# SarahAlkhateeb/Image-Captioning-with-Different-Decoders

Hardware: AMD Instinct MI355X
Metric: training images/sec (whole node), 'attention' decoder, at 1/2/4/8 MI355X (higher is better)
Workload: dtype fp32; 1 GPU; 'attention' decoder + frozen ResNet-101 encoder (BN train mode), one training step per batch; per_gpu_batch=64, global_batch=64, image_size=224, caption_len=25, decode_steps=24, vocab=8100, attention_dim=512, decoder_dim=512, embed_size=512, decoder_rows=49 distinct (AdaptiveAvgPool 7->14 replicate; exact, DESIGN.md 4.4), parallelism=dp1

## Files before the change

### image-captioning-with-different-decoders_amd/capmi/_lib.py

```python
import ctypes
import os

import torch

_HERE = os.path.dirname(os.path.abspath(__file__))
LIB_PATH = os.environ.get("CAPMI_LIB") or os.path.join(_HERE, "libcapmi.so")

c_int, c_ll, c_float, c_double, c_vp = ctypes.c_int, ctypes.c_longlong, ctypes.c_float, ctypes.c_double, ctypes.c_void_p
c_ull = ctypes.c_ulonglong

CAPMI_A_KMAJOR, CAPMI_A_MMAJOR, CAPMI_A_CONV_NHWC, CAPMI_A_CONV_NCHW, CAPMI_A_CONV_NHWC4 = 0, 1, 2, 3, 4
CAPMI_B_NMAJOR_W, CAPMI_B_KROWS, CAPMI_B_CONV_NHWC = 0, 1, 2
CAPMI_TILE_128, CAPMI_TILE_64, CAPMI_TILE_128x64, CAPMI_TILE_AUTO, CAPMI_TILE_128_W8 = 0, 1, 2, 3, 4
CAPMI_MAX_GROUP = 4
CAPMI_COLSUM_GROUPS = 64
ABI_VERSION = 27
CAPMI_BNB_RELU_Y, CAPMI_BNB_RELU_OUT = 0, 1
CAPMI_BNB_MAX_SLABS = 256
CAPMI_GEMM_BF16 = 1
CAPMI_GEMM_BF16_IO = 2
CAPMI_GEMM_X3 = 4
CAPMI_GEMM_X3P = 8
CAPMI_GEMM_SPLIT3 = 16
CAPMI_GEMM_X3D = 32
# ... 28 lines not shown

class DstepEpi(ctypes.Structure):
    _fields_ = [
        ("mode", c_int), ("out0", c_vp), ("ld0", c_ll), ("bias0", c_vp), ("nsplit", c_int),
        ("out1", c_vp), ("ld1", c_ll), ("bias1", c_vp), ("act1", c_int), ("D", c_int),
        ("xemb", c_vp), ("c_prev", c_vp), ("h_out", c_vp), ("c_out", c_vp), ("act_out", c_vp),
        ("dhd", c_vp), ("dc_in", c_vp), ("act", c_vp), ("c_cur", c_vp), ("dgates", c_vp), ("dc_out", c_vp),
        ("bt", c_int), ("gate", c_vp), ("awe", c_vp), ("dawe_out", c_vp), ("dgp", c_vp),
    ]


CAPMI_DSTEP_STORE2, CAPMI_DSTEP_LSTM_FWD, CAPMI_DSTEP_LSTM_BWD, CAPMI_DSTEP_GATE_BWD = 0, 1, 2, 3

_SIGS = {
    "capmi_gemm": [ctypes.POINTER(GemmProblem), c_int, c_int, c_int, c_int, c_vp],
    "capmi_gemm_stat_tiles": [c_int, c_int],
    "capmi_gemm_workspace_bytes": [],
    "capmi_gemm_workspace_flag_bytes": [],
    "capmi_gemm_sk": [ctypes.POINTER(GemmProblem), c_int, c_int, c_int, c_vp, c_ll, c_vp],
    "capmi_gemm_ex": [ctypes.POINTER(GemmProblem), c_int, c_int, c_int, c_int, c_int, c_vp],
    "capmi_gemm_sk_ex": [ctypes.POINTER(GemmProblem), c_int, c_int, c_int, c_int, c_vp, c_ll, c_vp],
    "capmi_gemm_sk_plan": [ctypes.POINTER(GemmProblem), c_int, c_int, c_int, c_int, c_vp, c_vp, c_vp, c_vp, c_vp],
    "capmi_last_launch_name": [ctypes.c_char_p, c_int],
    "capmi_splitk_reduce": [c_vp, c_int, c_ll, c_int, c_int, c_ll, c_vp, c_vp, c_ll, c_vp],
    "capmi_colsum": [c_vp, c_int, c_int, c_ll, c_float, c_vp, c_vp, c_int, c_vp],
    "capmi_conv_weight_pack": [c_vp, c_int, c_int, c_int, c_int, c_vp, c_vp],
    "capmi_conv_weight_pack_pad": [c_vp, c_int, c_int, c_int, c_int, c_int, c_vp, c_vp],
    "capmi_image_nhwc4": [c_vp, c_int, c_int, c_int, c_int, c_vp, c_vp],
    "capmi_bn_finalize": [c_vp, c_int, c_int, c_ll, c_vp, c_vp, c_vp, c_vp, c_float, c_float,
                          c_vp, c_vp, c_vp, c_vp, c_vp, c_vp],
    "capmi_bn_eval_params": [c_vp, c_vp, c_vp, c_vp, c_int, c_float, c_vp, c_vp, c_vp],
    "capmi_bn_add_relu": [c_vp, c_vp, c_vp, c_vp, c_vp, c_vp, c_vp, c_ll, c_int, c_vp],
    "capmi_bn_relu_maxpool": [c_vp, c_vp, c_vp, c_vp, c_int, c_int, c_int, c_int, c_int, c_int, c_vp],
    "capmi_adaptive_avgpool_nhwc": [c_vp, c_int, c_int, c_int, c_int, c_int, c_int, c_vp, c_vp],
    "capmi_conv_weight_pack_dgrad": [c_vp, c_int, c_int, c_int, c_int, c_vp, c_vp],
    "capmi_conv_weight_pack_dgrad_s2": [c_vp, c_int, c_int, c_int, c_int, c_vp, c_vp],
    "capmi_conv_weight_pack_dgrad_x3": [c_vp, c_int, c_int, c_int, c_int, c_int, c_int, c_vp, c_vp],
    "capmi_weight_x3_batch": [c_vp, c_int, c_ll, c_vp],
    "capmi_conv_weight_unpack": [c_vp, c_int, c_int, c_int, c_int, c_vp, c_vp],
    "capmi_zero_upsample2_nhwc": [c_vp, c_int, c_int, c_int, c_int, c_int, c_int, c_vp, c_vp],
    "capmi_bn_bwd_reduce": [c_int, c_vp, c_vp, c_vp, c_vp, c_vp, c_vp, c_vp, c_vp, c_float, c_ll, c_int,
                            c_vp, c_vp, c_int, c_vp, c_vp, c_vp],
    "capmi_bn_bwd_apply": [c_int, c_vp, c_vp, c_vp, c_vp, c_vp, c_vp, c_ll, c_int, c_vp, c_vp, c_vp],
    "capmi_adaptive_avgpool_bwd_nhwc": [c_vp, c_int, c_int, c_int, c_int, c_int, c_int, c_vp, c_vp],
    "capmi_embed_gather": [c_vp, c_int, c_int, c_vp, c_int, c_int, c_int, c_vp, c_ll, c_vp],
    "capmi_embed_dense": [c_vp, c_int, c_int, c_int, c_int, c_vp, c_ll, c_vp],
# ... 111 lines not shown
```

### image-captioning-with-different-decoders_amd/capmi/kernels.py

```python
import ctypes
import weakref

import torch

from ._lib import DstepEpi, DstepSeg
from ._lib import (CAPMI_A_CONV_NHWC, CAPMI_A_KMAJOR, CAPMI_A_MMAJOR, CAPMI_B_NMAJOR_W, CAPMI_BNB_MAX_SLABS, CAPMI_GEMM_BF16,
                   CAPMI_GEMM_BF16_IO, CAPMI_GEMM_X3, CAPMI_GEMM_X3P,
                   CAPMI_GEMM_SPLIT3, CAPMI_GEMM_X3C, CAPMI_GEMM_X3D, CAPMI_GEMM_X3S, CAPMI_GEMM_X3W,
                   CAPMI_COLSUM_GROUPS, CAPMI_TILE_128, CAPMI_TILE_64,
                   CAPMI_TILE_128x64, CAPMI_TILE_AUTO, GemmProblem, call, lib)

F32 = torch.float32


def ptr(t):
    return None if t is None else t.data_ptr()


def stream():
    return torch.cuda.current_stream().cuda_stream


def _cuda(*ts, dtype=F32):
    for t in ts:
# ... 169 lines not shown
    v = [ctypes.c_int(0) for _ in range(5)]
    call("capmi_gemm_sk_plan", ctypes.byref(prob), CAPMI_A_MMAJOR, bmode, CAPMI_TILE_AUTO, _x3w_flags(bf16),
         *[ctypes.byref(x) for x in v])
    return f"{'gemm_w16_kernel' if bf16 else 'gemm_x3w_kernel'}<{bmode}, {'true' if v[2].value else 'false'}>"


def gemm_x3w_ok(prob, bmode, bf16=False):
    v = [ctypes.c_int(0) for _ in range(5)]
    return lib.capmi_gemm_sk_plan(ctypes.byref(prob), CAPMI_A_MMAJOR, bmode, CAPMI_TILE_AUTO, _x3w_flags(bf16),
                                  *[ctypes.byref(x) for x in v]) == 0


def gemm_x3s_ok(prob, amode):
    v = [ctypes.c_int(0) for _ in range(5)]
    return lib.capmi_gemm_sk_plan(ctypes.byref(prob), amode, CAPMI_B_NMAJOR_W, CAPMI_TILE_AUTO, CAPMI_GEMM_X3S,
                                  *[ctypes.byref(x) for x in v]) == 0


def gemm_x3s_kernel_name(prob, amode):
    ncb = {64: 1, 128: 2, 256: 4}[prob.N]
    return f"gemm_x3s_kernel<{ncb}, {'true' if prob.in_scale else 'false'}>"


def gemm_x3d_kernel_name(prob, amode):
    v = [ctypes.c_int(0) for _ in range(5)]
    call("capmi_gemm_sk_plan", ctypes.byref(prob), amode, CAPMI_B_NMAJOR_W, CAPMI_TILE_AUTO, CAPMI_GEMM_X3D,
         *[ctypes.byref(x) for x in v])
    b = lambda x: "true" if x else "false"
    return f"gemm_x3p_kernel<{amode}, {b(v[2].value)}, 32, true, {b(bool(prob.in_scale))}>"


def gemm_x3p_kernel_name(prob, amode):
    v = [ctypes.c_int(0) for _ in range(5)]
    call("capmi_gemm_sk_plan", ctypes.byref(prob), amode, CAPMI_B_NMAJOR_W, CAPMI_TILE_AUTO, CAPMI_GEMM_X3P,
         *[ctypes.byref(x) for x in v])
    return f"gemm_x3p_kernel<{amode}, {'true' if v[2].value else 'false'}, {v[3].value}, false, false>"


def gemm_x3_kernel_name(prob, amode, tile=CAPMI_TILE_AUTO):
    v = [ctypes.c_int(0) for _ in range(5)]
    call("capmi_gemm_sk_plan", ctypes.byref(prob), amode, CAPMI_B_NMAJOR_W, tile, CAPMI_GEMM_X3,
         *[ctypes.byref(x) for x in v])
    b = lambda x: "true" if x else "false"
    return f"gemm_x3_kernel<{v[1].value}, {amode}, {b(bool(prob.in_scale))}, {b(v[2].value)}>"


# ... 621 lines not shown
```

### image-captioning-with-different-decoders_amd/capmi/resnet.py

```python
import os

import torch
import torch.nn as nn

from . import kernels as K
from ._lib import CAPMI_A_CONV_NHWC, CAPMI_A_CONV_NHWC4, CAPMI_A_KMAJOR, CAPMI_A_MMAJOR, CAPMI_B_CONV_NHWC
from ._lib import CAPMI_B_KROWS, CAPMI_B_NMAJOR_W, CAPMI_GEMM_BF16, CAPMI_GEMM_SPLIT3

AK, AMM, AC = CAPMI_A_KMAJOR, CAPMI_A_MMAJOR, CAPMI_A_CONV_NHWC
BW, BKR, BCONV = CAPMI_B_NMAJOR_W, CAPMI_B_KROWS, CAPMI_B_CONV_NHWC


class Bottleneck(nn.Module):
    expansion = 4

    def __init__(self, cin, width, stride=1, downsample=False):
        super().__init__()
        self.conv1 = nn.Conv2d(cin, width, 1, bias=False)
        self.bn1 = nn.BatchNorm2d(width)
        self.conv2 = nn.Conv2d(width, width, 3, stride=stride, padding=1, bias=False)
        self.bn2 = nn.BatchNorm2d(width)
        self.conv3 = nn.Conv2d(width, width * 4, 1, bias=False)
        self.bn3 = nn.BatchNorm2d(width * 4)
        self.relu = nn.ReLU(inplace=True)
# ... 70 lines not shown
        return ent[2]


def feature_hw(H, W):
    def down(x, k, st, pad):
        return (x + 2 * pad - k) // st + 1
    h, w = down(down(H, 7, 2, 3), 3, 2, 1), down(down(W, 7, 2, 3), 3, 2, 1)
    for _ in range(3):
        h, w = down(h, 3, 2, 1), down(w, 3, 2, 1)
    return h, w


def pool_dup(H, W, out_hw):
    fh, fw = feature_hw(H, W)
    oh, ow = out_hw
    if fh <= 0 or fw <= 0 or oh % fh or ow % fw or oh // fh != ow // fw:
        return 1
    return oh // fh


_X3_SMALLK = int(os.environ.get("CAPMI_X3_SMALLK", "0"))
_X3D = os.environ.get("CAPMI_X3D", "1") != "0"
_X3S = os.environ.get("CAPMI_X3S", "1") != "0"
_X3C = os.environ.get("CAPMI_X3C", "1") != "0"

class EncoderRunner:

    def __init__(self):
        self.packed = _Packed()
        self._ws = None
        self._ws_key = None
        self.conv_hook = None
        self.bf16 = False
        self.x3 = False

    def _workspace(self, N, H, W, device):
        key = (N, H, W, str(device))
        if self._ws_key != key:
            H1, W1 = (H + 6 - 7) // 2 + 1, (W + 6 - 7) // 2 + 1
            big = N * H1 * W1 * 64
            big = max(big, N * ((H1 + 1) // 2) * ((W1 + 1) // 2) * 256)
            f = dict(device=device, dtype=torch.float32)
            ws = {n: torch.empty(big, **f) for n in ("x", "y1", "y2", "y3", "yd", "out")}
            ws["stats"] = torch.empty(2 * ((N * H1 * W1 + 63) // 64) * 256, **f)
            ws["bnwork"] = torch.zeros(K.bn_work_doubles(2048), device=device, dtype=torch.float64)
            ws["ss"] = {}
            ws["sk"] = K.gemm_workspace(device)
            ws["img4"] = torch.empty(N * H * W * 4, **f)
            ws["x3p"] = None
            self._ws, self._ws_key = ws, key
        return self._ws

    def _x3p_buffer(self, ws):
        if ws["x3p"] is None:
            ws["x3p"] = torch.empty(3 * ws["x"].numel(), device=ws["x"].device, dtype=torch.bfloat16)
        return ws["x3p"]

# ... 122 lines not shown
            prob = K.problem(rows, co, Kd, x, ci, w, Kd, out, co, **kw_)
            mode = CAPMI_A_KMAJOR
        else:
            sc, sh = in_ss if in_ss is not None else (None, None)
            w = self._packed_x3(conv) if x3 and Kd % 32 == 0 and ci % 32 == 0 else self.packed.get(conv)
            prob = K.problem(rows, co, Kd, x, 0, w, Kd, out, co, conv=geo, in_scale=sc, in_shift=sh, **kw_)
            mode = CAPMI_A_CONV_NHWC
        if w.dtype == torch.bfloat16:
            launch = lambda: K.gemm_x3(prob, mode, self._ws["sk"])
            if self.conv_hook is not None:
                self.conv_hook(tag, 2.0 * rows * co * Kd, launch, K.gemm_x3_kernel_name(prob, mode))
            else:
                launch()
            return Ho, Wo, rows
        flags = CAPMI_GEMM_BF16 if self.bf16 else (CAPMI_GEMM_SPLIT3 if split3 else 0)
        launch = lambda: K.gemm_sk(prob, mode, self._ws["sk"], K.TILE_AUTO, flags=flags)
        if self.conv_hook is not None:
            key = K.gemm_sk_kernel_name(prob, mode, flags=flags)
            self.conv_hook(tag, 2.0 * rows * co * Kd, launch, key)
        else:
            launch()
        del stats
        return Ho, Wo, rows

    def _packed_x3(self, conv, tap_inner=False):
        w = conv.weight
        key = ("x3p" if tap_inner else "x3", id(conv))
        ent = self.packed.cache.get(key)
        if ent is None or ent[0] != w._version or ent[1] != w.data_ptr():
            src = self.packed.get(conv)
            if tap_inner:
                co, ci, kh, kw = w.shape
                src = K.conv_weight_order_x3p(src, kh, kw, ci)
            src = src.contiguous()
            dst = torch.empty(3 * src.numel(), device=w.device, dtype=torch.bfloat16)
            K.split3_bf16(src, dst)
            ent = (w._version, w.data_ptr(), dst)
            self.packed.cache[key] = ent
        return ent[2]

    def _packed_bf16(self, conv):
        w = conv.weight
        key = ("bf16", id(conv))
        ent = self.packed.cache.get(key)
        if ent is None or ent[0] != w._version or ent[1] != w.data_ptr():
            src = self.packed.get(conv).contiguous()
# ... 83 lines not shown
        N, C0, H, W = imgs.shape
        if self.bf16:
            return self._forward_bf16(net, imgs, out_hw, train, out)
        ws = self._workspace(N, H, W, imgs.device)
        H1, W1, rows = self._conv("conv1", imgs, net.conv1, ws["y1"], N, H, W, train, nchw=True)
        s, b = self._bn(ws, net.bn1, rows, train)
        Hp, Wp = (H1 + 2 - 3) // 2 + 1, (W1 + 2 - 3) // 2 + 1
        K.bn_relu_maxpool(ws["y1"], s, b, ws["x"], N, H1, W1, 64, Hp, Wp)
        x, xo = ws["x"], ws["out"]
        H, W, Cx = Hp, Wp, 64
        bns = []
        direct = out_hw is None and out is not None
        n4 = len(net.layer4)
        for li in range(1, 5):
            layer = getattr(net, f"layer{li}")
            for bi, blk in enumerate(layer):
                if direct and li == 4 and bi == n4 - 1:
                    xo = out
                tag = f"layer{li}.{bi}"
                _, _, r1 = self._conv(tag + ".conv1", x, blk.conv1, ws["y1"], N, H, W, train)
                ss1 = self._bn(ws, blk.bn1, r1, train)
                H2, W2, r2 = self._conv(tag + ".conv2", ws["y1"], blk.conv2, ws["y2"], N, H, W, train, in_ss=ss1)
                ss2 = self._bn(ws, blk.bn2, r2, train)
                _, _, r3 = self._conv(tag + ".conv3", ws["y2"], blk.conv3, ws["y3"], N, H2, W2, train, in_ss=ss2)
                Cout = blk.conv3.out_channels
                if blk.downsample is not None:
                    s3, b3 = self._bn(ws, blk.bn3, r3, train)
                    self._conv(tag + ".downsample", x, blk.downsample[0], ws["yd"], N, H, W, train)
                    sd, bd = self._bn(ws, blk.downsample[1], r3, train)
                    K.bn_add_relu(ws["y3"], s3, b3, ws["yd"], xo, r3, Cout, res_scale=sd, res_shift=bd)
                    bns.append(blk.downsample[1])
                else:
                    s3, b3 = self._bn(ws, blk.bn3, r3, train)
                    K.bn_add_relu(ws["y3"], s3, b3, x, xo, r3, Cout)
                bns += [blk.bn1, blk.bn2, blk.bn3]
                x, xo = xo, x
                H, W, Cx = H2, W2, Cout
        if train:
            bns.append(net.bn1)
            nbt = [m.num_batches_tracked for m in bns if m.num_batches_tracked is not None]
            if nbt:
                torch._foreach_add_(nbt, 1)
        if out_hw is None:
            return x if direct else x[: N * H * W * Cx].view(N, H, W, Cx).clone()
        OH, OW = out_hw
        if out is None:
            out = torch.empty(N, OH, OW, Cx, device=imgs.device, dtype=torch.float32)
        K.adaptive_avgpool_nhwc(x, N, H, W, Cx, OH, OW, out)
        return out


def conv_flops_per_image(net, H=224, W=224):
    tot = 0
    h, w = H, W
    convs = [net.conv1]
# ... 99 lines not shown
        for li in range(1, 5):
            for bi, blk in enumerate(getattr(net, f"layer{li}")):
                tag = f"layer{li}.{bi}"
                wd, Cout = blk.conv1.out_channels, blk.conv3.out_channels
                st = blk.conv2.stride[0]
                H2, W2 = (H + 2 - 3) // st + 1, (W + 2 - 3) // st + 1
                r1, r3 = N * H * W, N * H2 * W2
                if li < self.first:
                    y1, y2, y3, yd, o = ws["y1"], ws["y2"], ws["y3"], ws["yd"], xo
                else:
                    g = self.saved.get
                    y1 = g(tag + ".y1", r1 * wd, dev)
                    y2 = g(tag + ".y2", r3 * wd, dev)
                    y3 = g(tag + ".y3", r3 * Cout, dev)
                    yd = g(tag + ".yd", r3 * Cout, dev) if blk.downsample is not None else None
                    o = g(tag + ".out", r3 * Cout, dev)
                trainable = li >= self.first
                bnf = (lambda bn, rows: self._bn_save(ws, bn, rows)) if trainable else \
                    (lambda bn, rows: r._bn(ws, bn, rows, True) + (None,))
                r._conv(tag + ".conv1", x, blk.conv1, y1, N, H, W, True)
                s1, b1, m1 = bnf(blk.bn1, r1)
                r._conv(tag + ".conv2", y1, blk.conv2, y2, N, H, W, True, in_ss=(s1, b1))
                s2, b2, m2 = bnf(blk.bn2, r3)
                r._conv(tag + ".conv3", y2, blk.conv3, y3, N, H2, W2, True, in_ss=(s2, b2))
                s3, b3, m3 = bnf(blk.bn3, r3)
                md = sd = bd = None
                if blk.downsample is not None:
                    r._conv(tag + ".downsample", x, blk.downsample[0], yd, N, H, W, True)
                    sd, bd, md = bnf(blk.downsample[1], r3)
                    K.bn_add_relu(y3, s3, b3, yd, o, r3, Cout, res_scale=sd, res_shift=bd)
                    bns.append(blk.downsample[1])
                else:
                    K.bn_add_relu(y3, s3, b3, x, o, r3, Cout)
                bns += [blk.bn1, blk.bn2, blk.bn3]
                if trainable:
                    blocks.append(dict(blk=blk, tag=tag, li=li, x=x, Cin=Cx, H=H, W=W, H2=H2, W2=W2, wd=wd, Cout=Cout,
                                       stride=st, y1=y1, y2=y2, y3=y3, yd=yd, out=o,
                                       ss=[(s1, b1, m1), (s2, b2, m2), (s3, b3, m3), (sd, bd, md)]))
                    x = o
                else:
                    x, xo = o, x
                H, W, Cx = H2, W2, Cout
        nbt = [m.num_batches_tracked for m in bns if m.num_batches_tracked is not None]
        if nbt:
            torch._foreach_add_(nbt, 1)
        OH, OW = out_hw if out_hw is not None else (H, W)
        if out is None:
            out = torch.empty(N, OH, OW, Cx, device=dev, dtype=torch.float32)
        K.adaptive_avgpool_nhwc(x, N, H, W, Cx, OH, OW, out)
        self.state = dict(N=N, H=H, W=W, C=Cx, OH=OH, OW=OW, blocks=blocks, device=dev)
        return out

    def _flags(self, prob, amode, bmode):
        if not (self.r.x3 and _FT_DGRAD_X3):
            return 0
# ... 275 lines not shown
```

### image-captioning-with-different-decoders_amd/csrc/gemm.hip

```cpp
#include <cstdlib>

#include "common.h"

#include "gemm_args.h"

constexpr int BK = 16;

template <int AMODE> struct APad { static constexpr int v = 2; };
template <> struct APad<1> { static constexpr int v = 4; };
template <> struct APad<3> { static constexpr int v = 4; };
template <int BMODE> struct BPad { static constexpr int v = 2; };
template <> struct BPad<1> { static constexpr int v = 4; };

template <bool VEC>
__device__ __forceinline__ float4 load4(const float* p, int n) {
  if (VEC) {
    return n > 0 ? *reinterpret_cast<const float4*>(p) : make_float4(0.f, 0.f, 0.f, 0.f);
  } else {
    float4 v = make_float4(0.f, 0.f, 0.f, 0.f);
    if (n > 0) v.x = p[0];
    if (n > 1) v.y = p[1];
    if (n > 2) v.z = p[2];
    if (n > 3) v.w = p[3];
    return v;
// ... 1094 lines not shown
                CAPMI_ERANGE);
  CAPMI_REQUIRE(gemm_x3c_band_fits(p), CAPMI_EINVAL);
  tiles = (int)cdiv(p.M, 256);
  return 0;
}

int gemm_x3c(const capmi_gemm_problem* prob, int amode, int bmode, hipStream_t s) {
  int tiles = 0;
  const int rc = x3c_plan(prob, amode, bmode, tiles);
  if (rc) return rc;
  if (prob->M == 0) return 0;
  return gemm_x3c_launch(*prob, tiles, s);
}

int gemm_x3s(const capmi_gemm_problem* prob, int amode, int bmode, hipStream_t s) {
  long long lda = 0;
  int tiles = 0, grid = 0;
  const int rc = x3s_plan(prob, amode, bmode, lda, tiles, grid);
  if (rc) return rc;
  if (prob->M == 0) return 0;
  return gemm_x3s_launch(*prob, lda, tiles, grid, s);
}

int gemm_x3(const capmi_gemm_problem* prob, int amode, int bmode, int tile, void* workspace, long long ws_bytes,
            hipStream_t s) {
  GemmArgs a;
  int bn = 128;
  bool sk = false;
  long long total = 0;
  const int rc = x3_plan(prob, amode, bmode, tile, a, bn, sk, total);
  if (rc) return rc;
  if (prob->M == 0) return 0;
  if (!sk || workspace == nullptr) return gemm_x3_launch(a, amode, bn, (int)total, s);
  CAPMI_REQUIRE(aligned16(workspace), CAPMI_EINVAL);
  CAPMI_REQUIRE(ws_bytes >= capmi_gemm_workspace_bytes(), CAPMI_ERANGE);
  const int cus = cu_count();
  const long long slots = sk_cus();
  a.sk_nkt = prob->K / 32;
  a.sk_dp_tiles = sk_hybrid() && total >= 2 * slots ? (int)((total / slots - 1) * slots) : 0;
  a.sk_units = (total - a.sk_dp_tiles) * a.sk_nkt;
  a.sk_workers = (int)std::min<long long>(slots, a.sk_units);
  a.sk_groups = sk_xcd_groups() && a.sk_workers % 8 == 0 && total >= 64 ? 8 : 1;
  a.sk_flags = static_cast<int*>(workspace);
  a.sk_part = reinterpret_cast<float*>(static_cast<char*>(workspace) + sk_flag_bytes(cus));
  return gemm_x3_launch(a, amode, bn, a.sk_workers, s);
}
}

extern "C" int capmi_gemm_sk_ex(const capmi_gemm_problem* prob, int amode, int bmode, int tile, int flags,
                                void* workspace, long long ws_bytes, void* stream) {
  GemmPlan g;
  bool sk = false;
  if (flags == CAPMI_GEMM_BF16_IO) return gemm_bf16_io(prob, amode, bmode, tile, workspace, ws_bytes, as_stream(stream));
  if (flags == CAPMI_GEMM_X3) return gemm_x3(prob, amode, bmode, tile, workspace, ws_bytes, as_stream(stream));
  if (flags == CAPMI_GEMM_X3P) return gemm_x3p(prob, amode, bmode, workspace, ws_bytes, as_stream(stream));
  if (flags == CAPMI_GEMM_X3D) return gemm_x3d(prob, amode, bmode, workspace, ws_bytes, as_stream(stream));
  if (flags == CAPMI_GEMM_X3S) return gemm_x3s(prob, amode, bmode, as_stream(stream));
  if (flags == CAPMI_GEMM_X3W) return gemm_x3w(prob, amode, bmode, workspace, ws_bytes, as_stream(stream), 3);
  if (flags == (CAPMI_GEMM_X3W | CAPMI_GEMM_BF16))
    return gemm_x3w(prob, amode, bmode, workspace, ws_bytes, as_stream(stream), 1);
  if (flags == CAPMI_GEMM_X3C) return gemm_x3c(prob, amode, bmode, as_stream(stream));
  int terms = flag_terms(flags);
  CAPMI_REQUIRE(terms >= 0, CAPMI_EINVAL);
  CAPMI_REQUIRE(terms_mode_ok(terms, amode, bmode), CAPMI_EINVAL);
  int rc = sk_decide(prob, amode, bmode, tile, terms, g, sk);
  if (rc) return rc;
  if (terms > 0 && !(g.nt_ok && g.nt == 256 && (prob->in_scale == nullptr || amode == CAPMI_A_CONV_NHWC || bmode == CAPMI_B_CONV_NHWC))) {
    terms = 0;
    rc = sk_decide(prob, amode, bmode, tile, 0, g, sk);
    if (rc) return rc;
  }
// ... 93 lines not shown
```

### image-captioning-with-different-decoders_amd/csrc/gemm_args.h

```cpp
#pragma once
#include "common.h"

typedef float f32x16 __attribute__((ext_vector_type(16)));

struct GemmArgs {
  capmi_gemm_problem p[CAPMI_MAX_GROUP];
  int tiles_begin[CAPMI_MAX_GROUP + 1];
  int tiles_m[CAPMI_MAX_GROUP];
  int tiles_n[CAPMI_MAX_GROUP];
  int kchunk[CAPMI_MAX_GROUP];
  int nprob;
  int sk_workers;
  int sk_nkt;
  long long sk_units;
  int sk_dp_tiles;
  int sk_groups;
  float* sk_part;
  int* sk_flags;
  int tile_cols_first;
  int plain_epi;
  int x3d_pipe;
};

typedef float capmi_f32x2 __attribute__((ext_vector_type(2)));
// ... 43 lines not shown

__device__ __forceinline__ long long remap(long long r, long long r1, long long ld, long long s2) {
  return r1 > 0 ? (r % r1) * ld + (r / r1) * s2 : r * ld;
}

inline int plain_epilogue(const capmi_gemm_problem& p, int bn) {
  static const bool off = [] {
    const char* e = getenv("CAPMI_X3_PLAIN_EPI");
    return e && e[0] == '0';
  }();
  const bool ok = !off && p.alpha == 1.f && p.alpha_ptr == nullptr && p.bias == nullptr && p.bias2 == nullptr &&
                  !p.relu && p.c_r1 <= 0 && p.ksplit == 1 && p.N % bn == 0 && p.ldc >= p.N &&
                  (long long)p.M * p.ldc * 4 < (1LL << 31);
  return ok ? (p.beta == 0.f ? 1 : 2) : 0;
}

int gemm_nt_launch(const GemmArgs& a, int amode, int bmode, int bm, int bn, int blocks, hipStream_t s,
                   int terms = 0, int nt = 256);
int gemm_bf16_launch(const GemmArgs& a, int amode, int bm, int bn, int blocks, hipStream_t s, int stages);
int gemm_x3_launch(const GemmArgs& a, int amode, int bn, int blocks, hipStream_t s);
int gemm_x3p_launch(const GemmArgs& a, int amode, int bk, int blocks, hipStream_t s);
int gemm_x3d_launch(const GemmArgs& a, int amode, int blocks, hipStream_t s);
int gemm_x3s_launch(const capmi_gemm_problem& p, long long lda, int tiles, int grid, hipStream_t s);
int gemm_x3w_launch(const GemmArgs& a, int bmode, int blocks, hipStream_t s, int terms);
int gemm_x3c_launch(const capmi_gemm_problem& p, int tiles, hipStream_t s);
int gemm_x3c_max_width();
bool gemm_x3c_band_fits(const capmi_gemm_problem& p);
inline int gemm_nt_wg_per_cu(int bm, int bn, int terms = 0) {
  if (terms == 3) return bm == 64 && bn == 64 ? 2 : 1;
  return bm == 64 && bn == 64 ? 4 : 2;
}
```

### image-captioning-with-different-decoders_amd/csrc/gemm_x3s.hip

```cpp
#include "gemm_args.h"

namespace {

constexpr int SBM = 64;
constexpr int SKD = 64;
constexpr int SNT = 256;
typedef __bf16 bf16x8_s __attribute__((ext_vector_type(8)));
typedef __bf16 bf16x4_s __attribute__((ext_vector_type(4)));
typedef float f32x4_s __attribute__((ext_vector_type(4)));
constexpr unsigned kOOBs = 0x80000000u;

__device__ __forceinline__ __amdgpu_buffer_rsrc_t rsrc_s(const void* p, unsigned bytes) {
  return __builtin_amdgcn_make_buffer_rsrc(const_cast<void*>(p), 0, (int)bytes, 0x00020000);
}

__device__ __forceinline__ int soff(int r, int c) { return r * SKD + ((c ^ ((r >> 1) & 7)) << 3); }

__device__ __forceinline__ bf16x4_s cvt4s(float4 v) {
  bf16x4_s r;
  r.x = (__bf16)v.x;
  r.y = (__bf16)v.y;
  r.z = (__bf16)v.z;
  r.w = (__bf16)v.w;
  return r;
}

template <int NCB, bool PRO>
__global__ void __launch_bounds__(SNT) __attribute__((amdgpu_waves_per_eu(2)))
gemm_x3s_kernel(const capmi_gemm_problem P, long long lda, int tiles) {
  __shared__ __attribute__((aligned(16))) __bf16 As[2][3][SBM * SKD];
  const int tid = threadIdx.x, lane = tid & 63, wid = tid >> 6;
  const int rl = lane & 15, c4 = lane >> 4;
  const int M = P.M, N = P.N;
  const int wc0 = wid * 16 * NCB;

  bf16x8_s bw[NCB][2][3];
  {
    const long long plane = (long long)N * P.ldb;
    const auto rb = rsrc_s(P.B, (unsigned)(3 * plane * 2));
#pragma unroll
    for (int cb = 0; cb < NCB; ++cb)
#pragma unroll
      for (int kc = 0; kc < 2; ++kc)
#pragma unroll
        for (int p = 0; p < 3; ++p) {
          const unsigned off = (unsigned)((p * plane + (long long)(wc0 + 16 * cb + rl) * P.ldb + 32 * kc + 8 * c4) * 2);
          bw[cb][kc][p] = __builtin_bit_cast(bf16x8_s, __builtin_amdgcn_raw_buffer_load_b128(rb, off, 0, 0));
        }
  }
  const int ak = (tid & 15) * 4, ar = tid >> 4;
  float4 sc = f4(1.f), sh = f4(0.f);
  if (PRO) {
    sc = *reinterpret_cast<const float4*>(P.in_scale + ak);
// ... 11 lines not shown
      areg[s] = __builtin_bit_cast(
          float4, __builtin_amdgcn_raw_buffer_load_b128(ra, ok ? (unsigned)(row * lda + ak) * 4u : kOOBs, 0, 0));
      amsk |= (unsigned)ok << s;
    }
  };
  auto store_a = [&](int buf) {
#pragma unroll
    for (int s = 0; s < 4; ++s) {
      float4 v = areg[s];
      if (PRO) v = relu4(fma4(v, sc, sh));
      if (!((amsk >> s) & 1u)) v = f4(0.f);
      const bf16x4_s h0 = cvt4s(v);
      const float4 r1 = make_float4(v.x - (float)h0.x, v.y - (float)h0.y, v.z - (float)h0.z, v.w - (float)h0.w);
      const bf16x4_s h1 = cvt4s(r1);
      const bf16x4_s h2 = cvt4s(make_float4(r1.x - (float)h1.x, r1.y - (float)h1.y, r1.z - (float)h1.z,
                                            r1.w - (float)h1.w));
      const int o = soff(ar + 16 * s, ak >> 3) + (ak & 4);
      *reinterpret_cast<bf16x4_s*>(&As[buf][0][o]) = h0;
      *reinterpret_cast<bf16x4_s*>(&As[buf][1][o]) = h1;
      *reinterpret_cast<bf16x4_s*>(&As[buf][2][o]) = h2;
    }
  };

  int t = blockIdx.x;
  load_a(t);
  store_a(0);
  __syncthreads();
  const auto rc = rsrc_s(P.C, (unsigned)((long long)M * P.ldc * 4));
  const unsigned cbo = (unsigned)(wc0 + rl) * 4u;
  float* __restrict__ stats = P.stats;
  int buf = 0;
  for (; t < tiles; t += gridDim.x) {
    load_a(t + gridDim.x);
    __builtin_amdgcn_sched_barrier(0);
    f32x4_s acc[4][NCB];
#pragma unroll
    for (int rb = 0; rb < 4; ++rb) {
      bf16x8_s a[2][3];
#pragma unroll
      for (int kc = 0; kc < 2; ++kc)
#pragma unroll
        for (int p = 0; p < 3; ++p)
          a[kc][p] = *reinterpret_cast<const bf16x8_s*>(&As[buf][p][soff(16 * rb + rl, 4 * kc + c4)]);
#pragma unroll
      for (int cb = 0; cb < NCB; ++cb) {
        f32x4_s c = f32x4_s{0.f, 0.f, 0.f, 0.f};
#pragma unroll
        for (int kc = 0; kc < 2; ++kc) {
          c = __builtin_amdgcn_mfma_f32_16x16x32_bf16(a[kc][1], bw[cb][kc][1], c, 0, 0, 0);
          c = __builtin_amdgcn_mfma_f32_16x16x32_bf16(a[kc][0], bw[cb][kc][2], c, 0, 0, 0);
          c = __builtin_amdgcn_mfma_f32_16x16x32_bf16(a[kc][2], bw[cb][kc][0], c, 0, 0, 0);
          c = __builtin_amdgcn_mfma_f32_16x16x32_bf16(a[kc][0], bw[cb][kc][1], c, 0, 0, 0);
          c = __builtin_amdgcn_mfma_f32_16x16x32_bf16(a[kc][1], bw[cb][kc][0], c, 0, 0, 0);
          c = __builtin_amdgcn_mfma_f32_16x16x32_bf16(a[kc][0], bw[cb][kc][0], c, 0, 0, 0);
        }
        acc[rb][cb] = c;
      }
    }
    unsigned roff[4][4];
#pragma unroll
    for (int rb = 0; rb < 4; ++rb)
#pragma unroll
      for (int r = 0; r < 4; ++r) {
        const int row = t * SBM + 16 * rb + 4 * c4 + r;
        roff[rb][r] = row < M ? (unsigned)row * (unsigned)P.ldc * 4u : kOOBs;
      }
#pragma unroll
    for (int cb = 0; cb < NCB; ++cb) {
      float s = 0.f, q = 0.f;
#pragma unroll
      for (int rb = 0; rb < 4; ++rb)
#pragma unroll
        for (int r = 0; r < 4; ++r) {
          const float v = acc[rb][cb][r];
          __builtin_amdgcn_raw_buffer_store_b32(__float_as_uint(v), rc, roff[rb][r] + cbo + 64u * cb, 0, 0);
          s += v;
          q = fmaf(v, v, q);
        }
      if (stats != nullptr) {
        s += __shfl_xor(s, 16, 64);
        q += __shfl_xor(q, 16, 64);
        s += __shfl_xor(s, 32, 64);
        q += __shfl_xor(q, 32, 64);
        if (c4 == 0) {
          const long long o = ((long long)t * N + wc0 + 16 * cb + rl) * 2;
          *reinterpret_cast<float2*>(stats + o) = make_float2(s, q);
        }
      }
    }
    store_a(buf ^ 1);
    __syncthreads();
    buf ^= 1;
  }
}

}

int gemm_x3s_launch(const capmi_gemm_problem& p, long long lda, int tiles, int grid, hipStream_t s) {
  CAPMI_REQUIRE(grid >= 1 && grid <= tiles, CAPMI_EINVAL);
  const bool pro = p.in_scale != nullptr;
  const dim3 g(grid), b(SNT);
#define X3S_GO(NCB)                                                                    \
  do {                                                                                 \
    if (pro)                                                                           \
      CAPMI_KLAUNCH((gemm_x3s_kernel<NCB, true>), g, b, 0, s, p, lda, tiles);  \
    else                                                                      \
      CAPMI_KLAUNCH((gemm_x3s_kernel<NCB, false>), g, b, 0, s, p, lda, tiles); \
  } while (0)
  if (p.N == 64)
    X3S_GO(1);
  else if (p.N == 128)
    X3S_GO(2);
  else if (p.N == 256)
    X3S_GO(4);
  else
    return CAPMI_EINVAL;
#undef X3S_GO
  CAPMI_LAUNCH_CHECK();
  return 0;
}
```

### include/capmi.h

```cpp
#ifndef CAPMI_H
#define CAPMI_H

#ifdef __cplusplus
extern "C" {
#endif

#define CAPMI_ABI_VERSION 27

#define CAPMI_OK 0
#define CAPMI_EINVAL 1001
#define CAPMI_EALIGN 1002
#define CAPMI_ERANGE 1003

#define CAPMI_MAX_GROUP 4

enum capmi_amode {
  CAPMI_A_KMAJOR = 0,
  CAPMI_A_MMAJOR = 1,
  CAPMI_A_CONV_NHWC = 2,
  CAPMI_A_CONV_NCHW = 3,
  CAPMI_A_CONV_NHWC4 = 4
};
enum capmi_bmode {
  CAPMI_B_NMAJOR_W = 0,
// ... 23 lines not shown
int capmi_gemm(const capmi_gemm_problem* problems, int nprob, int amode, int bmode, int tile,
               void* stream);
int capmi_gemm_stat_tiles(int M, int tile);
long long capmi_gemm_workspace_bytes(void);
long long capmi_gemm_workspace_flag_bytes(void);
int capmi_gemm_sk(const capmi_gemm_problem* problem, int amode, int bmode, int tile, void* workspace,
                  long long ws_bytes, void* stream);
#define CAPMI_GEMM_BF16 1
#define CAPMI_GEMM_BF16_IO 2
#define CAPMI_GEMM_X3 4
#define CAPMI_GEMM_X3P 8
#define CAPMI_GEMM_X3D 32
#define CAPMI_GEMM_X3S 64
#define CAPMI_GEMM_X3W 128
#define CAPMI_GEMM_X3C 256
#define CAPMI_GEMM_SPLIT3 16
int capmi_gemm_ex(const capmi_gemm_problem* problems, int nprob, int amode, int bmode, int tile, int flags,
                  void* stream);
int capmi_gemm_sk_ex(const capmi_gemm_problem* problem, int amode, int bmode, int tile, int flags, void* workspace,
                     long long ws_bytes, void* stream);
int capmi_gemm_sk_plan(const capmi_gemm_problem* problem, int amode, int bmode, int tile, int flags, int* bm,
                       int* bn, int* stream_k, int* generic, int* threads);
int capmi_last_launch_name(char* out, int n);

int capmi_splitk_reduce(const float* in, int S, long long slab, int rows, int cols, long long ld_in,
                        const float* bias, float* out, long long ld_out, void* stream);
#define CAPMI_COLSUM_GROUPS 64
int capmi_colsum(const float* in, int rows, int cols, long long ld, float scale, float* work,
                 float* out, int accumulate, void* stream);

int capmi_conv_weight_pack(const float* w, int Cout, int Cin, int KH, int KW, float* out, void* stream);
int capmi_conv_weight_pack_pad(const float* w, int Cout, int Cin, int KH, int KW, int Cin_pad, float* out,
                               void* stream);
int capmi_image_nhwc4(const float* in, int N, int C, int H, int W, float* out, void* stream);
#define CAPMI_BN_WORK_DOUBLES(C) (64 + 64 * (long long)(C))
int capmi_bn_finalize(const float* stats, int tiles, int C, long long count, const float* gamma,
                      const float* beta, float* running_mean, float* running_var, float momentum,
                      float eps, float* scale, float* shift, float* save_mean, float* save_var,
                      void* work, void* stream);
int capmi_bn_eval_params(const float* gamma, const float* beta, const float* running_mean,
                         const float* running_var, int C, float eps, float* scale, float* shift,
                         void* stream);
int capmi_bn_relu_bf16(const void* y, const float* scale, const float* shift, long long rows, int C, void* x,
                       void* stream);
int capmi_bn_add_relu_bf16(const void* y, const float* scale, const float* shift, const void* res,
                           const float* res_scale, const float* res_shift, long long rows, int C, void* out,
// ... 224 lines not shown
```

Before: 6447 images/s.

## Fuse BN-add-ReLU into conv3 GEMM via stats pass plus recompute tail

For the 64->256 1x1 convolutions in the first ResNet stage, the conv output is no longer written to memory. A stats-only GEMM pass produces the BN statistics, and a second GEMM pass recomputes the product and applies BN, residual add and ReLU directly in the epilogue. This removes the write and re-read of the 256-channel intermediate and the separate bn_add_relu launch. The cost is doing the GEMM twice, and the path only applies to frozen or inference blocks with N=256.

```diff
diff --git a/image-captioning-with-different-decoders_amd/capmi/_lib.py b/image-captioning-with-different-decoders_amd/capmi/_lib.py
--- a/image-captioning-with-different-decoders_amd/capmi/_lib.py
+++ b/image-captioning-with-different-decoders_amd/capmi/_lib.py
@@ -74,6 +74,8 @@
     "capmi_gemm_sk_ex": [ctypes.POINTER(GemmProblem), c_int, c_int, c_int, c_int, c_vp, c_ll, c_vp],
     "capmi_gemm_sk_plan": [ctypes.POINTER(GemmProblem), c_int, c_int, c_int, c_int, c_vp, c_vp, c_vp, c_vp, c_vp],
     "capmi_last_launch_name": [ctypes.c_char_p, c_int],
+    "capmi_gemm_x3s_stats": [ctypes.POINTER(GemmProblem), c_int, c_vp],
+    "capmi_gemm_x3s_tail": [ctypes.POINTER(GemmProblem), c_int, c_vp, c_vp, c_vp, c_ll, c_vp, c_vp, c_int, c_vp],
     "capmi_splitk_reduce": [c_vp, c_int, c_ll, c_int, c_int, c_ll, c_vp, c_vp, c_ll, c_vp],
     "capmi_colsum": [c_vp, c_int, c_int, c_ll, c_float, c_vp, c_vp, c_int, c_vp],
     "capmi_conv_weight_pack": [c_vp, c_int, c_int, c_int, c_int, c_vp, c_vp],
diff --git a/image-captioning-with-different-decoders_amd/capmi/kernels.py b/image-captioning-with-different-decoders_amd/capmi/kernels.py
--- a/image-captioning-with-different-decoders_amd/capmi/kernels.py
+++ b/image-captioning-with-different-decoders_amd/capmi/kernels.py
@@ -215,6 +215,25 @@
     return f"gemm_x3s_kernel<{ncb}, {'true' if prob.in_scale else 'false'}>"
 
 
+def gemm_x3s_stats(prob, amode):
+    call("capmi_gemm_x3s_stats", ctypes.byref(prob), amode, stream())
+
+
+def gemm_x3s_tail(prob, amode, scale, shift, other, ld_other, res_scale=None, res_shift=None):
+    _cuda(scale, shift, other, res_scale, res_shift)
+    call("capmi_gemm_x3s_tail", ctypes.byref(prob), amode, ptr(scale), ptr(shift), ptr(other), int(ld_other),
+         ptr(res_scale), ptr(res_shift), int(res_scale is not None), stream())
+
+
+def gemm_x3s_stats_kernel_name(prob, amode):
+    return f"gemm_x3s_stats_kernel<4, {'true' if prob.in_scale else 'false'}>"
+
+
+def gemm_x3s_tail_kernel_name(prob, amode, acc_is_residual):
+    b = lambda x: "true" if x else "false"
+    return f"gemm_x3s_tail_kernel<4, {b(bool(prob.in_scale))}, {b(acc_is_residual)}>"
+
+
 def gemm_x3d_kernel_name(prob, amode):
     v = [ctypes.c_int(0) for _ in range(5)]
     call("capmi_gemm_sk_plan", ctypes.byref(prob), amode, CAPMI_B_NMAJOR_W, CAPMI_TILE_AUTO, CAPMI_GEMM_X3D,
diff --git a/image-captioning-with-different-decoders_amd/capmi/resnet.py b/image-captioning-with-different-decoders_amd/capmi/resnet.py
--- a/image-captioning-with-different-decoders_amd/capmi/resnet.py
+++ b/image-captioning-with-different-decoders_amd/capmi/resnet.py
@@ -116,6 +116,7 @@
 _X3_SMALLK = int(os.environ.get("CAPMI_X3_SMALLK", "0"))
 _X3D = os.environ.get("CAPMI_X3D", "1") != "0"
 _X3S = os.environ.get("CAPMI_X3S", "1") != "0"
+_X3S_TAIL = os.environ.get("CAPMI_X3S_TAIL", "1") != "0"
 _X3C = os.environ.get("CAPMI_X3C", "1") != "0"
 
 class EncoderRunner:
@@ -127,6 +128,7 @@
         self.conv_hook = None
         self.bf16 = False
         self.x3 = False
+        self.x3s_tail = _X3S_TAIL
 
     def _workspace(self, N, H, W, device):
         key = (N, H, W, str(device))
@@ -295,6 +297,42 @@
             launch()
         del stats
         return Ho, Wo, rows
+
+    def _conv_tail(self, tag, x, conv, bn, other, out, N, H, W, train, in_ss=None, main_ss=None):
+        co, ci, kh, kw = conv.weight.shape
+        rows = N * H * W
+        if not (self.x3s_tail and _X3S and self.x3 and ci == 64 and co == 256 and kh == 1 and kw == 1
+                and conv.stride[0] == 1 and conv.padding[0] == 0 and rows * co * 4 < (1 << 31)):
+            return False
+        w3 = self._packed_x3(conv)
+        stats = self._ws["stats"] if train else None
+        if in_ss is None:
+            prob, mode = K.problem(rows, co, ci, x, ci, w3, ci, out, co, stats=stats), CAPMI_A_KMAJOR
+        else:
+            geo = dict(N=N, H=H, W=W, Cin=ci, KH=1, KW=1, stride=1, pad=0, Ho=H, Wo=W)
+            prob = K.problem(rows, co, ci, x, 0, w3, ci, out, co, conv=geo, in_scale=in_ss[0], in_shift=in_ss[1],
+                             stats=stats)
+            mode = CAPMI_A_CONV_NHWC
+        if not K.gemm_x3s_ok(prob, mode):
+            return False
+
+        def run(tag, flops, launch, key):
+            if self.conv_hook is not None:
+                self.conv_hook(tag, flops, launch, key)
+            else:
+                launch()
+
+        if train:
+            run(tag, 2.0 * rows * co * ci, lambda: K.gemm_x3s_stats(prob, mode),
+                K.gemm_x3s_stats_kernel_name(prob, mode))
+        s, b = self._bn(self._ws, bn, rows, train)
+        res = main_ss is not None
+        if res:
+            tail = lambda: K.gemm_x3s_tail(prob, mode, main_ss[0], main_ss[1], other, co, s, b)
+        else:
+            tail = lambda: K.gemm_x3s_tail(prob, mode, s, b, other, co)
+        run(tag + ".tail", 0.0, tail, K.gemm_x3s_tail_kernel_name(prob, mode, res))
+        return True
 
     def _packed_x3(self, conv, tap_inner=False):
         w = conv.weight
@@ -424,15 +462,19 @@
                 ss1 = self._bn(ws, blk.bn1, r1, train)
                 H2, W2, r2 = self._conv(tag + ".conv2", ws["y1"], blk.conv2, ws["y2"], N, H, W, train, in_ss=ss1)
                 ss2 = self._bn(ws, blk.bn2, r2, train)
-                _, _, r3 = self._conv(tag + ".conv3", ws["y2"], blk.conv3, ws["y3"], N, H2, W2, train, in_ss=ss2)
                 Cout = blk.conv3.out_channels
                 if blk.downsample is not None:
+                    _, _, r3 = self._conv(tag + ".conv3", ws["y2"], blk.conv3, ws["y3"], N, H2, W2, train, in_ss=ss2)
                     s3, b3 = self._bn(ws, blk.bn3, r3, train)
-                    self._conv(tag + ".downsample", x, blk.downsample[0], ws["yd"], N, H, W, train)
-                    sd, bd = self._bn(ws, blk.downsample[1], r3, train)
-                    K.bn_add_relu(ws["y3"], s3, b3, ws["yd"], xo, r3, Cout, res_scale=sd, res_shift=bd)
+                    if not self._conv_tail(tag + ".downsample", x, blk.downsample[0], blk.downsample[1], ws["y3"],
+                                           xo, N, H, W, train, main_ss=(s3, b3)):
+                        self._conv(tag + ".downsample", x, blk.downsample[0], ws["yd"], N, H, W, train)
+                        sd, bd = self._bn(ws, blk.downsample[1], r3, train)
+                        K.bn_add_relu(ws["y3"], s3, b3, ws["yd"], xo, r3, Cout, res_scale=sd, res_shift=bd)
                     bns.append(blk.downsample[1])
-                else:
+                elif not self._conv_tail(tag + ".conv3", ws["y2"], blk.conv3, blk.bn3, x, xo, N, H2, W2, train,
+                                         in_ss=ss2):
+                    _, _, r3 = self._conv(tag + ".conv3", ws["y2"], blk.conv3, ws["y3"], N, H2, W2, train, in_ss=ss2)
                     s3, b3 = self._bn(ws, blk.bn3, r3, train)
                     K.bn_add_relu(ws["y3"], s3, b3, x, xo, r3, Cout)
                 bns += [blk.bn1, blk.bn2, blk.bn3]
@@ -578,15 +620,22 @@
                 s1, b1, m1 = bnf(blk.bn1, r1)
                 r._conv(tag + ".conv2", y1, blk.conv2, y2, N, H, W, True, in_ss=(s1, b1))
                 s2, b2, m2 = bnf(blk.bn2, r3)
-                r._conv(tag + ".conv3", y2, blk.conv3, y3, N, H2, W2, True, in_ss=(s2, b2))
-                s3, b3, m3 = bnf(blk.bn3, r3)
                 md = sd = bd = None
+                fused = not trainable and blk.downsample is None and r._conv_tail(
+                    tag + ".conv3", y2, blk.conv3, blk.bn3, x, o, N, H2, W2, True, in_ss=(s2, b2))
+                if not fused:
+                    r._conv(tag + ".conv3", y2, blk.conv3, y3, N, H2, W2, True, in_ss=(s2, b2))
+                    s3, b3, m3 = bnf(blk.bn3, r3)
+                    fused = not trainable and blk.downsample is not None and r._conv_tail(
+                        tag + ".downsample", x, blk.downsample[0], blk.downsample[1], y3, o, N, H, W, True,
+                        main_ss=(s3, b3))
                 if blk.downsample is not None:
-                    r._conv(tag + ".downsample", x, blk.downsample[0], yd, N, H, W, True)
-                    sd, bd, md = bnf(blk.downsample[1], r3)
-                    K.bn_add_relu(y3, s3, b3, yd, o, r3, Cout, res_scale=sd, res_shift=bd)
+                    if not fused:
+                        r._conv(tag + ".downsample", x, blk.downsample[0], yd, N, H, W, True)
+                        sd, bd, md = bnf(blk.downsample[1], r3)
+                        K.bn_add_relu(y3, s3, b3, yd, o, r3, Cout, res_scale=sd, res_shift=bd)
                     bns.append(blk.downsample[1])
-                else:
+                elif not fused:
                     K.bn_add_relu(y3, s3, b3, x, o, r3, Cout)
                 bns += [blk.bn1, blk.bn2, blk.bn3]
                 if trainable:
diff --git a/image-captioning-with-different-decoders_amd/csrc/gemm.hip b/image-captioning-with-different-decoders_amd/csrc/gemm.hip
--- a/image-captioning-with-different-decoders_amd/csrc/gemm.hip
+++ b/image-captioning-with-different-decoders_amd/csrc/gemm.hip
@@ -1140,6 +1140,21 @@
   return gemm_x3s_launch(*prob, lda, tiles, grid, s);
 }
 
+int x3s_pass_plan(const capmi_gemm_problem* prob, int amode, bool need_c, capmi_gemm_problem& p, long long& lda,
+                  int& tiles, int& grid) {
+  CAPMI_REQUIRE(prob != nullptr, CAPMI_EINVAL);
+  p = *prob;
+  if (!need_c && p.C == nullptr) {
+    p.C = const_cast<float*>(p.A);
+    p.ldc = p.N;
+  }
+  const int rc = x3s_plan(&p, amode, CAPMI_B_NMAJOR_W, lda, tiles, grid);
+  if (rc) return rc;
+  CAPMI_REQUIRE(p.N == 256, CAPMI_EINVAL);
+  if (!need_c) p.C = nullptr;
+  return 0;
+}
+
 int gemm_x3(const capmi_gemm_problem* prob, int amode, int bmode, int tile, void* workspace, long long ws_bytes,
             hipStream_t s) {
   GemmArgs a;
@@ -1165,6 +1180,36 @@
 }
 }
 
+extern "C" int capmi_gemm_x3s_stats(const capmi_gemm_problem* prob, int amode, void* stream) {
+  capmi_gemm_problem p;
+  long long lda = 0;
+  int tiles = 0, grid = 0;
+  const int rc = x3s_pass_plan(prob, amode, false, p, lda, tiles, grid);
+  if (rc) return rc;
+  CAPMI_REQUIRE(p.stats != nullptr, CAPMI_EINVAL);
+  if (p.M == 0) return 0;
+  return gemm_x3s_stats_launch(p, lda, tiles, grid, as_stream(stream));
+}
+
+extern "C" int capmi_gemm_x3s_tail(const capmi_gemm_problem* prob, int amode, const float* scale, const float* shift,
+                                   const float* other, long long ld_other, const float* res_scale,
+                                   const float* res_shift, int acc_is_residual, void* stream) {
+  capmi_gemm_problem p;
+  long long lda = 0;
+  int tiles = 0, grid = 0;
+  CAPMI_REQUIRE(scale && shift && other && (acc_is_residual == 0 || acc_is_residual == 1), CAPMI_EINVAL);
+  CAPMI_REQUIRE(acc_is_residual ? (res_scale && res_shift) : (!res_scale && !res_shift), CAPMI_EINVAL);
+  const int rc = x3s_pass_plan(prob, amode, true, p, lda, tiles, grid);
+  if (rc) return rc;
+  CAPMI_REQUIRE(aligned16(other), CAPMI_EALIGN);
+  CAPMI_REQUIRE(ld_other >= p.N && (long long)p.M * ld_other * 4 < (1LL << 31), CAPMI_EINVAL);
+  CAPMI_REQUIRE(((long long)p.M + 63) * std::max(ld_other, p.ldc) * 4 < (1LL << 32), CAPMI_ERANGE);
+  if (p.M == 0) return 0;
+  p.stats = nullptr;
+  const X3sTail e{scale, shift, other, ld_other, res_scale, res_shift};
+  return gemm_x3s_tail_launch(p, lda, tiles, grid, e, acc_is_residual != 0, as_stream(stream));
+}
+
 extern "C" int capmi_gemm_sk_ex(const capmi_gemm_problem* prob, int amode, int bmode, int tile, int flags,
                                 void* workspace, long long ws_bytes, void* stream) {
   GemmPlan g;
diff --git a/image-captioning-with-different-decoders_amd/csrc/gemm_args.h b/image-captioning-with-different-decoders_amd/csrc/gemm_args.h
--- a/image-captioning-with-different-decoders_amd/csrc/gemm_args.h
+++ b/image-captioning-with-different-decoders_amd/csrc/gemm_args.h
@@ -89,6 +89,17 @@
 int gemm_x3p_launch(const GemmArgs& a, int amode, int bk, int blocks, hipStream_t s);
 int gemm_x3d_launch(const GemmArgs& a, int amode, int blocks, hipStream_t s);
 int gemm_x3s_launch(const capmi_gemm_problem& p, long long lda, int tiles, int grid, hipStream_t s);
+struct X3sTail {
+  const float* scale;
+  const float* shift;
+  const float* other;
+  long long ld_other;
+  const float* res_scale;
+  const float* res_shift;
+};
+int gemm_x3s_stats_launch(const capmi_gemm_problem& p, long long lda, int tiles, int grid, hipStream_t s);
+int gemm_x3s_tail_launch(const capmi_gemm_problem& p, long long lda, int tiles, int grid, const X3sTail& e,
+                         bool acc_is_residual, hipStream_t s);
 int gemm_x3w_launch(const GemmArgs& a, int bmode, int blocks, hipStream_t s, int terms);
 int gemm_x3c_launch(const capmi_gemm_problem& p, int tiles, hipStream_t s);
 int gemm_x3c_max_width();
diff --git a/image-captioning-with-different-decoders_amd/csrc/gemm_x3s.hip b/image-captioning-with-different-decoders_amd/csrc/gemm_x3s.hip
--- a/image-captioning-with-different-decoders_amd/csrc/gemm_x3s.hip
+++ b/image-captioning-with-different-decoders_amd/csrc/gemm_x3s.hip
@@ -25,10 +25,13 @@
   return r;
 }
 
-template <int NCB, bool PRO>
-__global__ void __launch_bounds__(SNT) __attribute__((amdgpu_waves_per_eu(2)))
-gemm_x3s_kernel(const capmi_gemm_problem P, long long lda, int tiles) {
+enum { X3S_STORE = 0, X3S_STATS = 1, X3S_TAIL = 2, X3S_TAIL_RES = 3 };
+
+template <int NCB, bool PRO, int EPI>
+__device__ __forceinline__ void x3s_body(const capmi_gemm_problem& P, long long lda, int tiles, const X3sTail& E) {
+  constexpr bool kTail = EPI == X3S_TAIL || EPI == X3S_TAIL_RES;
   __shared__ __attribute__((aligned(16))) __bf16 As[2][3][SBM * SKD];
+  __shared__ float Bn[4][64 * NCB];
   const int tid = threadIdx.x, lane = tid & 63, wid = tid >> 6;
   const int rl = lane & 15, c4 = lane >> 4;
   const int M = P.M, N = P.N;
@@ -86,6 +89,16 @@
     }
   };
 
+  if constexpr (kTail) {
+    if (tid < 64 * NCB) {
+      Bn[0][tid] = E.scale[tid];
+      Bn[1][tid] = E.shift[tid];
+      if constexpr (EPI == X3S_TAIL_RES) {
+        Bn[2][tid] = E.res_scale[tid];
+        Bn[3][tid] = E.res_shift[tid];
+      }
+    }
+  }
   int t = blockIdx.x;
   load_a(t);
   store_a(0);
@@ -93,9 +106,34 @@
   const auto rc = rsrc_s(P.C, (unsigned)((long long)M * P.ldc * 4));
   const unsigned cbo = (unsigned)(wc0 + rl) * 4u;
   float* __restrict__ stats = P.stats;
+  float ov[16], bnp[4];
+  const auto ro = rsrc_s(E.other, (unsigned)((long long)M * E.ld_other * 4));
+  const unsigned ldo4 = (unsigned)E.ld_other * 4u, ldc4 = (unsigned)P.ldc * 4u;
+  unsigned obase = 0, cbase = 0;
+  auto load_o = [&](int cb) {
+    const int n = wc0 + rl + 16 * cb;
+    bnp[0] = Bn[0][n];
+    bnp[1] = Bn[1][n];
+    if constexpr (EPI == X3S_TAIL_RES) {
+      bnp[2] = Bn[2][n];
+      bnp[3] = Bn[3][n];
+    }
+    unsigned b = obase + 64u * cb;
+    asm volatile("" : "+v"(b));
+#pragma unroll
+    for (int k = 0; k < 16; ++k)
+      ov[k] = __uint_as_float(
+          __builtin_amdgcn_raw_buffer_load_b32(ro, b + (unsigned)(16 * (k >> 2) + (k & 3)) * ldo4, 0, 0));
+  };
   int buf = 0;
   for (; t < tiles; t += gridDim.x) {
     load_a(t + gridDim.x);
+    if constexpr (kTail) {
+      const unsigned row0 = (unsigned)(t * SBM + 4 * c4);
+      obase = row0 * ldo4 + cbo;
+      cbase = row0 * ldc4 + cbo;
+      load_o(0);
+    }
     __builtin_amdgcn_sched_barrier(0);
     f32x4_s acc[4][NCB];
 #pragma unroll
@@ -121,34 +159,61 @@
         acc[rb][cb] = c;
       }
     }
-    unsigned roff[4][4];
-#pragma unroll
-    for (int rb = 0; rb < 4; ++rb)
-#pragma unroll
-      for (int r = 0; r < 4; ++r) {
-        const int row = t * SBM + 16 * rb + 4 * c4 + r;
-        roff[rb][r] = row < M ? (unsigned)row * (unsigned)P.ldc * 4u : kOOBs;
-      }
-#pragma unroll
-    for (int cb = 0; cb < NCB; ++cb) {
-      float s = 0.f, q = 0.f;
-#pragma unroll
-      for (int rb = 0; rb < 4; ++rb)
-#pragma unroll
-        for (int r = 0; r < 4; ++r) {
-          const float v = acc[rb][cb][r];
-          __builtin_amdgcn_raw_buffer_store_b32(__float_as_uint(v), rc, roff[rb][r] + cbo + 64u * cb, 0, 0);
-          s += v;
-          q = fmaf(v, v, q);
-        }
-      if (stats != nullptr) {
-        s += __shfl_xor(s, 16, 64);
-        q += __shfl_xor(q, 16, 64);
-        s += __shfl_xor(s, 32, 64);
-        q += __shfl_xor(q, 32, 64);
-        if (c4 == 0) {
-          const long long o = ((long long)t * N + wc0 + 16 * cb + rl) * 2;
-          *reinterpret_cast<float2*>(stats + o) = make_float2(s, q);
+    if constexpr (kTail) {
+#pragma unroll
+      for (int cb = 0; cb < NCB; ++cb) {
+        unsigned b = cbase + 64u * cb;
+        asm volatile("" : "+v"(b));
+#pragma unroll
+        for (int rb = 0; rb < 4; ++rb)
+#pragma unroll
+          for (int r = 0; r < 4; ++r) {
+            const float v = acc[rb][cb][r], x = ov[4 * rb + r];
+            float o;
+            if constexpr (EPI == X3S_TAIL)
+              o = fmaxf(fmaf(v, bnp[0], bnp[1]) + x, 0.f);
+            else {
+              float rr = fmaf(v, bnp[2], bnp[3]);
+              asm("" : "+v"(rr));
+              o = fmaxf(fmaf(x, bnp[0], bnp[1]) + rr, 0.f);
+            }
+            __builtin_amdgcn_raw_buffer_store_b32(__float_as_uint(o), rc, b + (unsigned)(16 * rb + r) * ldc4, 0, 0);
+          }
+        if (cb + 1 < NCB) load_o(cb + 1);
+      }
+    } else {
+      unsigned roff[4][4];
+      if constexpr (EPI == X3S_STORE) {
+#pragma unroll
+        for (int rb = 0; rb < 4; ++rb)
+#pragma unroll
+          for (int r = 0; r < 4; ++r) {
+            const int row = t * SBM + 16 * rb + 4 * c4 + r;
+            roff[rb][r] = row < M ? (unsigned)row * (unsigned)P.ldc * 4u : kOOBs;
+          }
+      }
+#pragma unroll
+      for (int cb = 0; cb < NCB; ++cb) {
+        float s = 0.f, q = 0.f;
+#pragma unroll
+        for (int rb = 0; rb < 4; ++rb)
+#pragma unroll
+          for (int r = 0; r < 4; ++r) {
+            const float v = acc[rb][cb][r];
+            if constexpr (EPI == X3S_STORE)
+              __builtin_amdgcn_raw_buffer_store_b32(__float_as_uint(v), rc, roff[rb][r] + cbo + 64u * cb, 0, 0);
+            s += v;
+            q = fmaf(v, v, q);
+          }
+        if (stats != nullptr) {
+          s += __shfl_xor(s, 16, 64);
+          q += __shfl_xor(q, 16, 64);
+          s += __shfl_xor(s, 32, 64);
+          q += __shfl_xor(q, 32, 64);
+          if (c4 == 0) {
+            const long long o = ((long long)t * N + wc0 + 16 * cb + rl) * 2;
+            *reinterpret_cast<float2*>(stats + o) = make_float2(s, q);
+          }
         }
       }
     }
@@ -156,6 +221,24 @@
     __syncthreads();
     buf ^= 1;
   }
+}
+
+template <int NCB, bool PRO>
+__global__ void __launch_bounds__(SNT) __attribute__((amdgpu_waves_per_eu(2)))
+gemm_x3s_kernel(const capmi_gemm_problem P, long long lda, int tiles) {
+  x3s_body<NCB, PRO, X3S_STORE>(P, lda, tiles, X3sTail{});
+}
+
+template <int NCB, bool PRO>
+__global__ void __launch_bounds__(SNT) __attribute__((amdgpu_waves_per_eu(2)))
+gemm_x3s_stats_kernel(const capmi_gemm_problem P, long long lda, int tiles) {
+  x3s_body<NCB, PRO, X3S_STATS>(P, lda, tiles, X3sTail{});
+}
+
+template <int NCB, bool PRO, bool RES>
+__global__ void __launch_bounds__(SNT) __attribute__((amdgpu_waves_per_eu(2)))
+gemm_x3s_tail_kernel(const capmi_gemm_problem P, long long lda, int tiles, const X3sTail E) {
+  x3s_body<NCB, PRO, RES ? X3S_TAIL_RES : X3S_TAIL>(P, lda, tiles, E);
 }
 
 }
@@ -183,3 +266,34 @@
   CAPMI_LAUNCH_CHECK();
   return 0;
 }
+
+int gemm_x3s_stats_launch(const capmi_gemm_problem& p, long long lda, int tiles, int grid, hipStream_t s) {
+  CAPMI_REQUIRE(grid >= 1 && grid <= tiles && p.N == 256 && p.stats != nullptr, CAPMI_EINVAL);
+  const dim3 g(grid), b(SNT);
+  if (p.in_scale != nullptr)
+    CAPMI_KLAUNCH((gemm_x3s_stats_kernel<4, true>), g, b, 0, s, p, lda, tiles);
+  else
+    CAPMI_KLAUNCH((gemm_x3s_stats_kernel<4, false>), g, b, 0, s, p, lda, tiles);
+  CAPMI_LAUNCH_CHECK();
+  return 0;
+}
+
+int gemm_x3s_tail_launch(const capmi_gemm_problem& p, long long lda, int tiles, int grid, const X3sTail& e,
+                         bool acc_is_residual, hipStream_t s) {
+  CAPMI_REQUIRE(grid >= 1 && grid <= tiles && p.N == 256, CAPMI_EINVAL);
+  const bool pro = p.in_scale != nullptr;
+  const dim3 g(grid), b(SNT);
+  if (acc_is_residual) {
+    if (pro)
+      CAPMI_KLAUNCH((gemm_x3s_tail_kernel<4, true, true>), g, b, 0, s, p, lda, tiles, e);
+    else
+      CAPMI_KLAUNCH((gemm_x3s_tail_kernel<4, false, true>), g, b, 0, s, p, lda, tiles, e);
+  } else {
+    if (pro)
+      CAPMI_KLAUNCH((gemm_x3s_tail_kernel<4, true, false>), g, b, 0, s, p, lda, tiles, e);
+    else
+      CAPMI_KLAUNCH((gemm_x3s_tail_kernel<4, false, false>), g, b, 0, s, p, lda, tiles, e);
+  }
+  CAPMI_LAUNCH_CHECK();
+  return 0;
+}
diff --git a/include/capmi.h b/include/capmi.h
--- a/include/capmi.h
+++ b/include/capmi.h
@@ -69,6 +69,10 @@
 int capmi_gemm_sk_plan(const capmi_gemm_problem* problem, int amode, int bmode, int tile, int flags, int* bm,
                        int* bn, int* stream_k, int* generic, int* threads);
 int capmi_last_launch_name(char* out, int n);
+int capmi_gemm_x3s_stats(const capmi_gemm_problem* problem, int amode, void* stream);
+int capmi_gemm_x3s_tail(const capmi_gemm_problem* problem, int amode, const float* scale, const float* shift,
+                        const float* other, long long ld_other, const float* res_scale, const float* res_shift,
+                        int acc_is_residual, void* stream);
 
 int capmi_splitk_reduce(const float* in, int S, long long slab, int rows, int cols, long long ld_in,
                         const float* bias, float* out, long long ld_out, void* stream);
```

Result: faster. 6539 images/s, median of 6 (+1.4%).
